# bluemoon-o2/walker-gym

Hardware: AMD Instinct MI355X
Metric: env-steps/sec (whole node) at 65 536 walkers; 1/2/4/8 MI355X scaling (higher is better)
Workload: dtype f32

## Files before the change

include/walker_hip.h:

```cpp
#ifndef WALKER_HIP_H
#define WALKER_HIP_H
#include <stdint.h>

#ifdef __cplusplus
extern "C" {
#endif

typedef struct ihipStream_t *hipStream_t;
typedef struct ihipEvent_t *hipEvent_t;

#define WG_ABI_VERSION 16
#define WG_EINVAL (-1)
#define WG_ERANGE (-2)
#define WG_EHIP (-3)

typedef struct wg_params {
    double g, dampk, ground, groundk, grounddamp, friction, dt;
    double pk, vk, ak, mk;
    int32_t in3d, max_steps;
    int32_t midform;
    int32_t conmid;
    int32_t spring_mode;
    int32_t action_mode;
    int32_t integrator;
// ... 136 lines not shown
    int32_t n_sets, obs_dim, hidden, act_dim;
    uint64_t seed;
    uint32_t generation;
    float sigma;
    const float *theta;
    float *w1, *b1, *w2, *b2;
} wg_es;

int wg_es_perturb(const wg_es *es, int32_t first_pair, int32_t n_pairs, hipStream_t stream);
int wg_es_update(const wg_es *es, int32_t first_pair, int32_t n_pairs, const float *util, double scale, float lr,
                 double *workspace, float *grad, float *theta_out, hipStream_t stream);

typedef struct wg_range {
    const wg_batch *batch;
    const wg_outputs *outputs;
    int64_t action_offset;
    const int32_t *plan;
    int32_t plan_blocks;
    hipStream_t stream;
} wg_range;

int wg_step_ranges(const wg_range *ranges, int32_t n, const wg_params *p, const float *action, int32_t action_cols,
                   int32_t action_stride, hipEvent_t *events);

int wg_run_ranges(const wg_range *ranges, int32_t n, const wg_params *p, const float *action, int32_t action_cols,
                  int32_t action_stride, int64_t action_step, int32_t n_steps, hipEvent_t *events);

int wg_observe(const wg_batch *b, const wg_params *p, const wg_outputs *o, const int32_t *plan,
               int32_t plan_blocks, hipStream_t stream);

typedef wg_params wg_obs_cfg;
int wg_step_simple(const wg_batch *b, const float *action, const wg_params *p, int32_t n_steps, hipStream_t stream);
int wg_observe_simple(const wg_batch *b, const wg_obs_cfg *cfg, float *obs, float *reward, uint8_t *done,
                      float *centroid, float *energy, hipStream_t stream);

int wg_reset(const wg_batch *b, const wg_params *p, const float *noise, const uint8_t *mask,
             hipStream_t stream);

int wg_reset_noise(const wg_batch *b, const float *noise, hipStream_t stream);

int wg_plan_ragged(const int32_t *mass_off, const int32_t *edge_off, const int32_t *muscle_off,
                   int32_t N, int32_t *plan, int32_t max_blocks);

int wg_plan_waves(const int32_t *mass_off, const int32_t *edge_off, const int32_t *muscle_off,
                  int32_t N, int32_t *plan, int32_t max_tiles);
int wg_wave_edge_passes(int32_t M, int32_t K);

int wg_plan_errors(int32_t clear);

int wg_launch_geometry(const wg_batch *b, wg_launch_info *info);

long long wg_fix_launches(void);

int wg_debug_stamps(unsigned long long *host, int n);

int wg_launch_floor(int32_t mode, int32_t blocks, int32_t threads, const float *in, float *out, int32_t n_launches,
                    hipStream_t stream);

int wg_time_step(const wg_batch *batch, const wg_params *params, const float *action, int32_t action_cols,
                 int32_t action_stride, int64_t action_step, const wg_outputs *out, int32_t n_steps,
                 const int32_t *plan, int32_t plan_blocks, hipStream_t stream, float *ms_per_launch);

#ifdef __cplusplus
}
#endif
#endif
```

walker_gym_amd/_lib.py:

```python
from __future__ import annotations

import ctypes as C
import os
import threading

HERE = os.path.dirname(os.path.abspath(__file__))
LIB_NAME = "libwalker_hip.so"
LIB_PATH = os.path.join(HERE, LIB_NAME)
ABI_VERSION = 16

WG_EINVAL, WG_ERANGE, WG_EHIP = -1, -2, -3

_vp = C.c_void_p


class WgParams(C.Structure):
    _fields_ = [(n, C.c_double) for n in ("g", "dampk", "ground", "groundk", "grounddamp", "friction", "dt",
                                           "pk", "vk", "ak", "mk")] + \
               [(n, C.c_int32) for n in ("in3d", "max_steps", "midform", "conmid", "spring_mode", "action_mode",
                                         "integrator", "pair_mode")] + \
               [(n, C.c_double) for n in ("pair_g", "pair_k", "pair_e", "bounce_k")] + \
               [("g3_gravity", C.c_double * 3)] + \
               [(n, C.c_double) for n in ("g3_damping", "g3_air", "g3_ground_level", "g3_restitution",
                                          "g3_friction")] + [("g3_ground", C.c_int32), ("friction_mode", C.c_int32),
# ... 15 lines not shown
                ("reset_noise", _vp), ("reset_noise_rows", C.c_int32), ("reset_noise_stride", C.c_int64),
                ("episodes", _vp)]


class WgOutputs(C.Structure):
    _fields_ = [("obs", _vp), ("obs_stride", C.c_int32), ("reward", _vp), ("done", _vp),
                ("centroid", _vp), ("energy", _vp), ("obs_step", C.c_int64), ("out_step", C.c_int64),
                ("obs_pad_clean", C.c_int32), ("steps", _vp), ("nonfinite", _vp), ("momentum", _vp),
                ("reset", _vp), ("final_obs", _vp)]


class WgRange(C.Structure):
    _fields_ = [("batch", C.POINTER(WgBatch)), ("outputs", C.POINTER(WgOutputs)), ("action_offset", C.c_int64),
                ("plan", _vp), ("plan_blocks", C.c_int32), ("stream", _vp)]


class WgLaunchInfo(C.Structure):
    _fields_ = [("threads", C.c_int32), ("walkers_per_block", C.c_int32), ("blocks", C.c_int32),
                ("lds_bytes", C.c_int32)]


class WgPolicy(C.Structure):
    _fields_ = [("n_sets", C.c_int32), ("obs_dim", C.c_int32), ("hidden", C.c_int32), ("act_dim", C.c_int32),
                ("w1", _vp), ("b1", _vp), ("w2", _vp), ("b2", _vp), ("act_limit", C.c_float),
                ("action_out", _vp), ("action_out_step", C.c_int64), ("return_out", _vp), ("length_out", _vp)]


class WgEpisodeStats(C.Structure):
    _fields_ = [("return_sum", _vp), ("length_sum", _vp), ("episodes_done", _vp), ("tail_return", _vp),
                ("tail_length", _vp), ("ep_return", _vp), ("ep_length", _vp), ("ep_slots", C.c_int32)]


class WgEs(C.Structure):
    _fields_ = [("n_sets", C.c_int32), ("obs_dim", C.c_int32), ("hidden", C.c_int32), ("act_dim", C.c_int32),
                ("seed", C.c_uint64), ("generation", C.c_uint32), ("sigma", C.c_float), ("theta", _vp),
                ("w1", _vp), ("b1", _vp), ("w2", _vp), ("b2", _vp)]


class WgActionNoise(C.Structure):
    _fields_ = [("seed", C.c_uint64), ("step_base", C.c_uint32), ("walker_base", C.c_uint32), ("sigma", _vp),
                ("raw_out", _vp), ("raw_out_step", C.c_int64), ("eps_out", _vp), ("eps_out_step", C.c_int64)]


class WgPolicyRows(C.Structure):
    _fields_ = [("x", _vp), ("x_step", C.c_int64), ("mask", _vp), ("mask_step", C.c_int64), ("n_steps", C.c_int32),
                ("N", C.c_int32)]


POLICY_GRAD_MAX_K = 16384

EXPORTS = ("wg_abi_version", "wg_last_error", "wg_step", "wg_step_ranges", "wg_run_ranges", "wg_rollout", "wg_observe",
           "wg_step_simple", "wg_observe_simple", "wg_reset", "wg_reset_noise", "wg_plan_ragged", "wg_plan_waves",
           "wg_wave_edge_passes", "wg_plan_errors", "wg_launch_geometry", "wg_launch_floor", "wg_time_step",
           "wg_rollout_policy", "wg_rollout_episodes", "wg_fix_launches", "wg_es_perturb", "wg_es_update",
           "wg_rollout_stochastic", "wg_gae", "wg_policy_forward", "wg_policy_backward_workspace", "wg_policy_backward")

_lib = None
_lock = threading.Lock()


class WalkerHipError(RuntimeError):
    pass


def load(path: str | None = None):
    global _lib
    with _lock:
        if _lib is not None:
            return _lib
        p = path or os.environ.get("WALKER_HIP_LIB", LIB_PATH)
        if not os.path.exists(p):
            raise WalkerHipError(
                f"{p} not found: build it with `python -m walker_gym_amd.build` (hipcc --offload-arch=gfx950); "
                "walker_gym_amd has no CPU fallback")
        L = C.CDLL(p)
        L.wg_abi_version.restype = C.c_int
        L.wg_last_error.restype = C.c_char_p
        L.wg_step.argtypes = [C.POINTER(WgBatch), C.POINTER(WgParams), _vp, C.c_int32, C.c_int32, C.c_int64,
                              C.POINTER(WgOutputs), C.c_int32, _vp, C.c_int32, _vp]
        L.wg_rollout.argtypes = L.wg_step.argtypes
        L.wg_rollout_policy.argtypes = [C.POINTER(WgBatch), C.POINTER(WgParams), C.POINTER(WgPolicy),
                                        C.POINTER(WgOutputs), C.c_int32, _vp]
        L.wg_rollout_episodes.argtypes = [C.POINTER(WgBatch), C.POINTER(WgParams), C.POINTER(WgPolicy),
                                          C.POINTER(WgOutputs), C.POINTER(WgEpisodeStats), C.c_int32, _vp]
        L.wg_rollout_stochastic.argtypes = [C.POINTER(WgBatch), C.POINTER(WgParams), C.POINTER(WgPolicy),
                                            C.POINTER(WgActionNoise), C.POINTER(WgOutputs), C.POINTER(WgEpisodeStats),
                                            C.c_int32, _vp]
        L.wg_gae.argtypes = [_vp, _vp, _vp, _vp, _vp, C.c_int32, C.c_int32, C.c_int64, C.c_float, C.c_float, _vp, _vp,
                             _vp]
        L.wg_policy_forward.argtypes = [C.POINTER(WgPolicy), C.POINTER(WgPolicyRows), _vp, C.c_int64, _vp]
        L.wg_policy_backward_workspace.argtypes = [C.POINTER(WgPolicy), C.POINTER(WgPolicyRows), C.c_int32]
        L.wg_policy_backward.argtypes = [C.POINTER(WgPolicy), C.POINTER(WgPolicyRows), _vp, C.c_int64, C.c_int32, _vp,
                                         _vp, _vp, _vp, _vp, _vp]
        L.wg_es_perturb.argtypes = [C.POINTER(WgEs), C.c_int32, C.c_int32, _vp]
        L.wg_es_update.argtypes = [C.POINTER(WgEs), C.c_int32, C.c_int32, _vp, C.c_double, C.c_float, _vp, _vp, _vp, _vp]
        L.wg_step_ranges.argtypes = [C.POINTER(WgRange), C.c_int32, C.POINTER(WgParams), _vp, C.c_int32, C.c_int32,
                                     C.POINTER(_vp)]
        L.wg_run_ranges.argtypes = [C.POINTER(WgRange), C.c_int32, C.POINTER(WgParams), _vp, C.c_int32, C.c_int32,
                                    C.c_int64, C.c_int32, C.POINTER(_vp)]
        L.wg_observe.argtypes = [C.POINTER(WgBatch), C.POINTER(WgParams), C.POINTER(WgOutputs), _vp, C.c_int32, _vp]
        L.wg_step_simple.argtypes = [C.POINTER(WgBatch), _vp, C.POINTER(WgParams), C.c_int32, _vp]
        L.wg_observe_simple.argtypes = [C.POINTER(WgBatch), C.POINTER(WgParams), _vp, _vp, _vp, _vp, _vp, _vp]
        L.wg_reset.argtypes = [C.POINTER(WgBatch), C.POINTER(WgParams), _vp, _vp, _vp]
        L.wg_reset_noise.argtypes = [C.POINTER(WgBatch), _vp, _vp]
        L.wg_plan_ragged.argtypes = [_vp, _vp, _vp, C.c_int32, _vp, C.c_int32]
        L.wg_plan_waves.argtypes = [_vp, _vp, _vp, C.c_int32, _vp, C.c_int32]
        L.wg_wave_edge_passes.argtypes = [C.c_int32, C.c_int32]
        L.wg_plan_errors.argtypes = [C.c_int32]
        L.wg_launch_geometry.argtypes = [C.POINTER(WgBatch), C.POINTER(WgLaunchInfo)]
        L.wg_launch_floor.argtypes = [C.c_int32, C.c_int32, C.c_int32, _vp, _vp, C.c_int32, _vp]
        L.wg_time_step.argtypes = L.wg_step.argtypes + [C.POINTER(C.c_float)]
        for f in EXPORTS[2:]:
            getattr(L, f).restype = C.c_int
        L.wg_fix_launches.restype = C.c_longlong
        L.wg_policy_backward_workspace.restype = C.c_int64
        v = L.wg_abi_version()
        if v != ABI_VERSION:
            raise WalkerHipError(f"{p}: ABI version {v}, expected {ABI_VERSION}")
        _lib = L
        return L


def ptr(t):
    return None if t is None else C.c_void_p(t.data_ptr())


def check(rc: int, what: str) -> int:
    if rc < 0:
        msg = load().wg_last_error().decode(errors="replace")
        exc = ValueError if rc in (WG_EINVAL, WG_ERANGE) else WalkerHipError
        raise exc(f"{what}: {msg} (code {rc})")
    return rc
```

walker_gym_amd/csrc/walker_hip.hip:

```cpp

#include <hip/hip_runtime.h>
#include <hip/hip_ext.h>

#include <algorithm>
#include <atomic>
#include <cstdarg>
#include <cstdint>
#include <cstdio>
#include <cstdlib>
#include <cstring>
#include <type_traits>
#include <vector>

#include "walker_hip.h"
#include "powf2.h"
#include "walker_internal.h"
#include "wg_philox.h"

static thread_local char g_err[512] = "";

int wg_fail(int code, const char *fmt, ...) {
    va_list ap;
    va_start(ap, fmt);
    vsnprintf(g_err, sizeof g_err, fmt, ap);
// ... 1896 lines not shown
        const double e = (b.charge && is_mass) ? b.charge[pl] : kp.pair_e;
        pair_central(kp.pair_k, e, p3, mf, lane, M, is_mass, ax, ay, az, true);
    }
}



typedef TermsAoS LeanTerms;
__device__ __forceinline__ LeanTerms lean_terms(char *sl, const LeanGeo &lg) {
    return TermsAoS{reinterpret_cast<double *>(sl), reinterpret_cast<float *>(sl + lg.off_df)};
}

template <bool IN3D, bool FIX = false>
__device__ __forceinline__ void lean_obs_rows(float *obs, int stride, const KParams &kp, int M, int A, int w0, int wl,
                                              int q, int mu_wl, int mu_ua, bool mass_on, bool mus_on, float px, float py,
                                              float pz, float vx, float vy, float vz, float ax, float ay, float az,
                                              float sx, float sy, float sz, float midx, float midy, float midz, float x) {
    constexpr int d = IN3D ? 3 : 2, per = 3 * d;
    const int nmid = (!FIX && kp.conmid) ? 3 : 0;
    typedef float fvd __attribute__((ext_vector_type(d), aligned(4)));
    if (mass_on) {
        const uint32_t row0 = (uint32_t)(w0 + wl) * (uint32_t)stride;
        const bool sums = !FIX && kp.midform == 2;
        const float mm[3] = {sums ? sx : midx, sums ? sy : midy, sums ? sz : midz};
        const float pm[3] = {px, py, pz}, vm[3] = {vx, vy, vz}, am[3] = {ax, ay, az};
        fvd vp, vv, va;
#pragma unroll
        for (int c = 0; c < d; c++) {
            if constexpr (FIX) {
                vp[c] = pm[c] - mm[c]; vv[c] = vm[c]; va[c] = am[c];
            } else {
                vp[c] = kp.midform ? (pm[c] - mm[c]) * kp.pk : pm[c] * kp.pk;
                vv[c] = vm[c] * kp.vk;
                va[c] = am[c] * kp.ak;
            }
        }
        float *dst = WG_ST(obs, row0 + per * q, 1);
        *reinterpret_cast<fvd *>(dst) = vp;
        *reinterpret_cast<fvd *>(dst + d) = vv;
        *reinterpret_cast<fvd *>(dst + 2 * d) = va;
        if (q == 0) {
            if (nmid) {
                float *mrow = WG_ST(obs, row0 + per * M, 1);
                mrow[0] = kp.midform ? mm[0] : 0.f; mrow[1] = kp.midform ? mm[1] : 0.f;
                mrow[2] = kp.midform ? mm[2] : 0.f;
            }
            for (int r = per * M + nmid + A; r < stride; r++) *WG_ST(obs, row0 + r, 1) = 0.f;
        }
    }
    if (mus_on)
        *WG_ST(obs, (uint32_t)(w0 + mu_wl) * (uint32_t)stride + per * M + nmid + mu_ua, 1) = FIX ? x : x * kp.mk;
}

__device__ __forceinline__ KParams lean_fix_params(KParams kp) {
    kp.pk = 1.f; kp.vk = 1.f; kp.ak = 1.f; kp.mk = 1.f;
    kp.midform = 1; kp.conmid = 0; kp.action_mode = 0; kp.integrator = 0; kp.pair_mode = 0;
    return kp;
}
struct LeanPolOut { float ax, ay, az, sx, sy, sz, reward; int done; int reset; };
template <bool IN3D, int NE, bool RES = false, bool E8 = false, bool AR = false, bool POL = false, bool FIX = false>
__device__ __forceinline__ void lean_compute(const wg_batch &b, const KParams &kp_in, const KOut &o,
                                             const LeanGeo &lg, char *sl, const LeanTile &t, int lane,
                                             LeanIn<NE, E8> &L, bool last = true, const KReset &ar = KReset{},
                                             LeanPolOut *po = nullptr, uint32_t *epw = nullptr, int epw_stride = 1) {
    static_assert(!FIX || (E8 && !RES && !AR && !POL && NE <= 4), "FIX: the plain E8 step instance");
    const KParams kp_fix = FIX ? lean_fix_params(kp_in) : KParams{};
    const KParams &kp = FIX ? kp_fix : kp_in;
    const bool store = !RES || last;
    const int M = b.M, K = b.K, A = b.A;
    const int w0 = t.w0, nE = t.nE;
    const int wl = t.wl, q = t.q, mu_wl = t.mu_wl, mu_ua = t.mu_ua;
    const bool is_mass = FIX || t.is_mass, is_mus = t.is_mus, acts = FIX ? t.is_mus : t.acts;
    const uint32_t pl = t.P0 + lane, ul = t.U0 + lane;
    const LeanTerms ts = lean_terms(sl, lg);
    STAMP_WAVE(t.w0 / lg.wpw);
    uint32_t *s_inc = reinterpret_cast<uint32_t *>(sl + lg.off_inc);
    float *s_x = reinterpret_cast<float *>(sl + lg.off_x);
    const float mf = L.mf;
    const bool pin = !FIX && L.pin != 0;
    double sq_tl = 0.0, sq_te = 0.0;
    if (NE == 1 && !RES) {
        sq_tl = PW_LOG2_TAB[lane & 31];
        sq_te = pw_asdouble(PW_EXP2_TAB[lane & 31]);
    }

    if (!RES) {
        WG_INC_TO_LDS(s_inc, L.gi, lane, nE, NE, FIX);
        if (lane == 0) s_inc[nE] = 0u;
    }
    float x = L.x;
    if (acts) {
        x = muscle_act(kp.action_mode, x, L.a, L.stp, L.lo, L.hi);
        if (store) *WG_ST(b.muscle_x, ul, 1) = x;
    }
    if (is_mus) s_x[lane] = x;
    double ym = recip_m(mf);
    if (!RES) asm volatile("" : "+v"(ym));
    wave_sync();
    STAMP(2);

    bool dead = false;
    if ((!RES || NE == 1) && kp.pair_mode == 0) {
        const bool nanp = is_mass && (__builtin_isnan(L.p3[0]) || __builtin_isnan(L.p3[1]) || __builtin_isnan(L.p3[2]));
        if (__builtin_expect(__ballot(nanp) != 0ull, 0)) {
            const unsigned long long db = __ballot(nanp && !pin && L.io1 > L.io0);
            const unsigned long long gm = (M == 64) ? ~0ull : (((1ull << M) - 1ull) << (lane & ~(M - 1)));
            dead = is_mass && (db & gm) == gm;
            if (dead) {
                L.p3[0] = (float)q; L.p3[1] = 0.f; L.p3[2] = 0.f;
                L.v3[0] = 0.f; L.v3[1] = 0.f; L.v3[2] = 0.f;
            }
        }
    }

    bool gtiny = false;
    const bool pos_ok = __all(fexp3(L.p3[0], L.p3[1], L.p3[2]) >= -55);
    struct Gath { float v[12]; };
    auto gather = [&](int it, Gath &g) {
// ... 51 lines not shown
            const int le = lane + 64 * it;
            if (le < nE) ts.put(le, 0.0, 0.0, 0.0, 0.f, 0.f, 0.f);
            continue;
        }
        Gath g;
        gather(it, g);
        spring(it, g);
    }
    wave_sync();
    const bool wave_tiny = __any(gtiny);
    STAMP(3);

    EnvTerms et{};
    if (!RES) et = env_terms(kp, mf, (float)ym, L.v3[0], L.v3[1], L.v3[2]);
    float px = 0.f, py = 0.f, pz = 0.f, vx = 0.f, vy = 0.f, vz = 0.f, ax = 0.f, ay = 0.f, az = 0.f;
    float nv = 0.f, ke = 0.f, pe = 0.f;
    bool hit = false;
    if (is_mass) {
        const int r1 = (WG_ABLATE & 2) ? min(L.io1, L.io0 + 1) : L.io1;
        const int lb = wl * K;
        if (!RES)
            mass_accumulate_v2(ts, reinterpret_cast<const uint16_t *>(s_inc) + 2 * lb, lb, L.io0, r1, mf, ym, ax, ay, az,
                               wave_tiny);
        else
            mass_accumulate<LeanTerms, !RES>(ts, reinterpret_cast<const uint16_t *>(s_inc) + 2 * lb, lb, L.io0, r1, mf,
                                             ax, ay, az, 0, wave_tiny);
    }
    if (!RES && kp.pair_mode) pair_forces(b, kp, L.p3, mf, pl, lane, M, is_mass, ax, ay, az);
    if (is_mass) {
        mass_tail(kp, mf, (float)ym, L.p3, L.v3, px, py, pz, vx, vy, vz, ax, ay, az, hit, pin,
                  !RES ? &et : nullptr);
        if (dead) nan_state(px, py, pz, vx, vy, vz, ax, ay, az, hit);
        if (!FIX && b.radius && store) b.radius[pl] = hit ? 3.0 : 1.0;
        nv = np_norm3(vx, vy, vz);
        if (!(NE == 1 && !RES)) ke = dead ? nv : mf * np_sq<NE == 1>(nv);
        pe = (float)((double)mf * kp.g) * (py - kp.ground);
    }
    if (NE == 1 && !RES) {
        const float sq = np_sq_wave(dead ? 0.f : nv, sq_tl, sq_te);
        if (is_mass) ke = dead ? nv : mf * sq;
    }
    STAMP(4);

    const int gbase = lane & ~(M - 1);
    const WalkerSums ws = (WG_ABLATE & 4) ? WalkerSums{px, py, pz, py, nv, ke, pe}
                                          : walker_sums(px, py, pz, nv, ke, pe, gbase, M, lane);
    const float sx = ws.sx, sy = ws.sy, sz = ws.sz, ysum = ws.ysum, vsum = ws.vsum, ksum = ws.ksum, psum = ws.psum;
    const unsigned long long gmask = (M == 64) ? ~0ull : (((1ull << M) - 1ull) << gbase);
    const unsigned long long hb = __ballot(is_mass && (py - kp.ground < 0.f));
    const unsigned long long sb = __ballot(is_mass && nv < 0.1f);
    const float midx = sx * lg.invM, midy = sy * lg.invM, midz = sz * lg.invM;
    int ep_done = 0;
    if (is_mass) {
        if (store) WG_STORE_STATE(b, pl, px, py, pz, vx, vy, vz, ax, ay, az, RES || kp.keep_aux, hit)
        if (q == 0) {
            const uint32_t wg = (uint32_t)(w0 + wl);
            const int steps = L.wsteps + 1;
            if (store) *WG_ST(b.steps, wg, 1) = steps;
            if (RES) L.wsteps = steps;
            if (o.steps) *WG_ST(o.steps, wg, 1) = steps;
            const float cy = ysum * lg.invM;
            if constexpr (POL) {
                const float vpen = (-(vsum * lg.invM)) * 0.1f;
                po->reward = (cy + vpen) + neg_half_count((int)__popcll(hb & gmask));
                if (o.reward) *WG_ST(o.reward, wg, 1) = po->reward;
            } else if (FIX || o.reward) {
                const float vpen = (-(vsum * lg.invM)) * 0.1f;
                *WG_ST(o.reward, wg, 1) = (cy + vpen) + neg_half_count((int)__popcll(hb & gmask));
            }
            if (FIX || o.done || (AR && (ar.mode & 1)) || POL) {
                int done;
                WG_EPISODE_DONE(done, steps, cy, (sb & gmask) == gmask, kp);
                if (FIX || o.done) at_u32w(o.done, wg) = (uint8_t)done;
                ep_done = done;
            }
            if (FIX || o.centroid) {
                float *c = WG_ST(o.centroid, wg, 3);
                c[0] = midx; c[1] = midy; c[2] = midz;
            }
            if (FIX || o.energy) *WG_ST(o.energy, wg, 1) = 0.5f * ksum + psum;
        }
    }

    STAMP(5);
    if ((FIX || o.obs) && !(WG_ABLATE & 16))
        lean_obs_rows<IN3D, FIX>(o.obs, o.obs_stride, kp, M, A, w0, wl, q, mu_wl, mu_ua, is_mass, is_mus, px, py, pz,
                                 vx, vy, vz, ax, ay, az, sx, sy, sz, midx, midy, midz, x);
    float rsx = sx, rsy = sy, rsz = sz;
    if constexpr (AR) {
        const bool nonf = is_mass && !(__builtin_isfinite(px) && __builtin_isfinite(py) && __builtin_isfinite(pz) &&
                                       __builtin_isfinite(vx) && __builtin_isfinite(vy) && __builtin_isfinite(vz) &&
                                       __builtin_isfinite(ax) && __builtin_isfinite(ay) && __builtin_isfinite(az));
        const unsigned long long eb = __ballot(is_mass && q == 0 && ep_done != 0), nb = __ballot(nonf);
        const unsigned long long hot = ((ar.mode & 1) ? eb : 0ull) | ((ar.mode & 2) ? nb : 0ull);
        const bool selw = is_mass && (hot & gmask) != 0ull;
        if (ar.reset && is_mass && q == 0) at_u32w(ar.reset, (uint32_t)(w0 + wl)) = (uint8_t)selw;
        if constexpr (POL) po->reset = selw;
        if (__builtin_expect(hot != 0ull, 0)) {
            const unsigned long long mmask = (M == 64) ? ~0ull : (((1ull << M) - 1ull) << ((mu_wl << lg.lgM) & 63));
            const bool selm = is_mus && (hot & mmask) != 0ull;
            if (ar.final_obs)
                lean_obs_rows<IN3D>(ar.final_obs, o.obs_stride, kp, M, A, w0, wl, q, mu_wl, mu_ua, selw, selm, px, py, pz,
                                    vx, vy, vz, ax, ay, az, sx, sy, sz, midx, midy, midz, x);
            int ep = 0;
            if (selw && q == 0) ep = RES ? (int)epw[wl * epw_stride] : at_u32(b.episodes, 4u * (uint32_t)(w0 + wl));
            ep = __builtin_amdgcn_ds_bpermute(gbase << 2, ep);
            float fx = px, fy = py, fz = pz, fvx = vx, fvy = vy, fvz = vz, fax = ax, fay = ay, faz = az, fxm = x;
            if (selw) {
                const float *ip = &at_u32(b.init_pos, 12u * pl), *iv = &at_u32(b.init_vel, 12u * pl),
                            *ia = &at_u32(b.init_acc, 12u * pl);
                fx = ip[0]; fy = ip[1]; fz = ip[2];
                fvx = iv[0]; fvy = iv[1]; fvz = iv[2];
                fax = ia[0]; fay = ia[1]; faz = ia[2];
                if (b.reset_noise) {
                    const float *nz = b.reset_noise +
                                      (size_t)((uint32_t)ep % (uint32_t)b.reset_noise_rows) * (size_t)b.reset_noise_stride +
                                      3 * (size_t)pl;
                    fvx = fvx + nz[0]; fvy = fvy + nz[1];
                    if (IN3D) fvz = fvz + nz[2];
                }
                if (store) {
                    float *gpo = WG_ST(b.pos, pl, 3), *gvo = WG_ST(b.vel, pl, 3), *gao = WG_ST(b.acc, pl, 3);
                    gpo[0] = fx; gpo[1] = fy; gpo[2] = fz;
                    gvo[0] = fvx; gvo[1] = fvy; gvo[2] = fvz;
                    gao[0] = fax; gao[1] = fay; gao[2] = faz;
                }
                if (q == 0) {
                    const uint32_t wg = (uint32_t)(w0 + wl);
                    if (store) *WG_ST(b.steps, wg, 1) = 0;
                    *WG_ST(b.episodes, wg, 1) = ep + 1;
                    if constexpr (RES) {
                        epw[wl * epw_stride] = (uint32_t)(ep + 1);
                        L.wsteps = 0;
                    }
                }
            }
            if (selm) {
                fxm = at_u32(b.init_muscle_x, 4u * ul);
                *WG_ST(b.muscle_x, ul, 1) = fxm;
            }
            if (o.obs && !(WG_ABLATE & 16)) {
                const WalkerSums fs = walker_sums(fx, fy, fz, 0.f, 0.f, 0.f, gbase, M, lane);
                lean_obs_rows<IN3D>(o.obs, o.obs_stride, kp, M, A, w0, wl, q, mu_wl, mu_ua, selw, selm, fx, fy, fz, fvx,
                                    fvy, fvz, fax, fay, faz, fs.sx, fs.sy, fs.sz, fs.sx * lg.invM, fs.sy * lg.invM,
                                    fs.sz * lg.invM, fxm);
            }
            if constexpr (RES) {
                px = fx; py = fy; pz = fz; vx = fvx; vy = fvy; vz = fvz; x = fxm;
                if constexpr (POL) {
                    const WalkerSums fs = walker_sums(fx, fy, fz, 0.f, 0.f, 0.f, gbase, M, lane);
                    ax = fax; ay = fay; az = faz;
                    if (selw) { rsx = fs.sx; rsy = fs.sy; rsz = fs.sz; }
                }
            }
        }
    }
    if (RES) {
        L.p3[0] = px; L.p3[1] = py; L.p3[2] = pz;
        L.v3[0] = vx; L.v3[1] = vy; L.v3[2] = vz;
        L.x = x;
    }
    if constexpr (POL) {
        po->ax = ax; po->ay = ay; po->az = az;
        po->sx = rsx; po->sy = rsy; po->sz = rsz;
        po->done = ep_done;
    }
    STAMP(6);
    STAMP_HW(lane);
}

constexpr int lean_waves(int NE) { return NE >= 8 ? 4 : 6; }

template <bool IN3D, int NE, bool E8, bool AR = false, bool FIX = false>
__global__ __launch_bounds__(256) __attribute__((amdgpu_waves_per_eu(lean_waves(NE)))) void walker_step_lean(
    typename std::conditional<AR, wg_batch, KBatch15>::type bk, KParams kp, const float *__restrict__ action,
    int action_cols, int action_stride, KOut o, LeanGeo lg, typename std::conditional<AR, KReset, KNoReset>::type ar) {
    extern __shared__ __attribute__((aligned(16))) char smem[];
    const wg_batch b = batch_of(bk);
    const int lane = threadIdx.x & 63, wv = __builtin_amdgcn_readfirstlane(threadIdx.x >> 6);
    const int blk = (kp.xcd & 2) ? xcd_block(blockIdx.x, gridDim.x) : (int)blockIdx.x;
    const int tile = blk * lg.wpb + wv;
    if (tile * lg.wpw >= b.N) return;
    STAMP_WAVE(tile);
    STAMP(0);
    const LeanTile t = lean_tile_of<FIX>(b, action, action_cols, lg, tile, lane);
    LeanIn<NE, E8> L;
    if (kp.prio) __builtin_amdgcn_s_setprio(2);
    lean_load<NE, E8, FIX>(b, kp, action, action_stride, t, lane, L);
    if (kp.prio) __builtin_amdgcn_s_setprio(0);
    STAMP(1);
    if constexpr (AR) lean_compute<IN3D, NE, false, E8, true>(b, kp, o, lg, smem + wv * lg.slice, t, lane, L, true, ar);
    else lean_compute<IN3D, NE, false, E8, false, false, FIX>(b, kp, o, lg, smem + wv * lg.slice, t, lane, L);
}

template <bool IN3D, bool E8, bool AR = false, bool FIX = false>
__global__ __launch_bounds__(256) __attribute__((amdgpu_waves_per_eu(lean_waves(1)))) void walker_step_lean1(
    float *pos, float *vel, const void *edges, const uint16_t *inc, int N, int M, int K, int wpw, int wpb, int nblkx,
    wg_batch b, KParams kp, const float *__restrict__ action, int action_cols, int action_stride, KOut o, LeanGeo lg,
    typename std::conditional<AR, KReset, KNoReset>::type ar) {
    extern __shared__ __attribute__((aligned(16))) char smem[];
    b.pos = pos; b.vel = vel; b.inc = inc; b.N = N; b.M = M; b.K = K;
    if (E8) b.edges8 = static_cast<const wg_edge8 *>(edges);
    else b.edges = static_cast<const wg_edge *>(edges);
    lg.nblk = nblkx & 0x3fffffff; lg.wpw = wpw; lg.wpb = wpb;
    kp.prio = (int)((unsigned)nblkx >> 31);
    const int lane = threadIdx.x & 63, wv = __builtin_amdgcn_readfirstlane(threadIdx.x >> 6);
    const int bid = blockIdx.x, xb = xcd_block(bid, lg.nblk);
    const int blk = (nblkx & 0x40000000) ? xb : bid;
    const int tile = blk * lg.wpb + wv;
    if (tile * lg.wpw >= b.N) return;
    STAMP_WAVE(tile);
    STAMP(0);
    const LeanTile t = lean_tile_of<FIX>(b, action, action_cols, lg, tile, lane);
    LeanIn<1, E8> L;
    if (kp.prio) __builtin_amdgcn_s_setprio(2);
    lean_load<1, E8, FIX>(b, kp, action, action_stride, t, lane, L);
    if (kp.prio) __builtin_amdgcn_s_setprio(0);
    STAMP(1);
    if constexpr (AR) lean_compute<IN3D, 1, false, E8, true>(b, kp, o, lg, smem + wv * lg.slice, t, lane, L, true, ar);
    else lean_compute<IN3D, 1, false, E8, false, false, FIX>(b, kp, o, lg, smem + wv * lg.slice, t, lane, L);
}

struct KResetRes {
    KReset r;
    int off_ep;
};
__device__ __forceinline__ KReset kreset_at(const KReset &r, const KOut &o, int s) {
    KReset as = r;
    if (as.reset) as.reset += (size_t)s * o.out_step;
    if (as.final_obs) as.final_obs += (size_t)s * o.obs_step;
    return as;
}
#define WG_KOUT_AT(os, o, s)                                          \
    KOut os = o;                                                      \
    if (os.obs) os.obs += (size_t)s * os.obs_step;                    \
    if (os.reward) os.reward += (size_t)s * os.out_step;              \
    if (os.done) os.done += (size_t)s * os.out_step;                  \
    if (os.energy) os.energy += (size_t)s * os.out_step;              \
    if (os.centroid) os.centroid += 3 * (size_t)s * os.out_step;      \
    if (os.steps) os.steps += (size_t)s * os.out_step
#define WG_PIN_STATIC(L, NE, E8)                                                                                      \
    {                                                                                                                 \
        asm volatile("" : "+v"(L.mf), "+v"(L.io0), "+v"(L.io1), "+v"(L.lo), "+v"(L.hi), "+v"(L.stp));                 \
        _Pragma("unroll") for (int it = 0; it < NE; it++) {                                                           \
            if constexpr (E8) asm volatile("" : "+v"(L.er[it].w), "+v"(L.er[it].rest));                               \
// ... 776 lines not shown
}

int wg_plan_waves(const int32_t *mass_off, const int32_t *edge_off, const int32_t *muscle_off, int32_t N,
                  int32_t *plan, int32_t max_tiles) {
    if (!mass_off || !edge_off || !muscle_off || !plan || N < 0 || max_tiles < 1)
        return wg_fail(WG_EINVAL, "bad plan args");
    int Mmax = 1, Kmax = 0;
    for (int w = 0; w < N; w++) {
        Mmax = std::max(Mmax, mass_off[w + 1] - mass_off[w]);
        Kmax = std::max(Kmax, edge_off[w + 1] - edge_off[w]);
    }
    const int ne = wave_passes(Mmax, Kmax);
    if (!ne) return wg_fail(WG_EINVAL, "a walker does not fit one wave (M=%d K=%d)", Mmax, Kmax);
    return pack_plan(mass_off, edge_off, muscle_off, N, plan, max_tiles, PackCaps{64, 64 * ne, 64, RW_MAXW}, true, "tiles");
}

int wg_plan_ragged(const int32_t *mass_off, const int32_t *edge_off, const int32_t *muscle_off,
                   int32_t N, int32_t *plan, int32_t max_blocks) {
    if (!mass_off || !edge_off || !muscle_off || !plan || N < 0 || max_blocks < 1)
        return wg_fail(WG_EINVAL, "bad plan args");
    return pack_plan(mass_off, edge_off, muscle_off, N, plan, max_blocks, PackCaps{RAG_P, RAG_E, RAG_U, RAG_W}, false,
                     "blocks");
}

int wg_launch_floor(int32_t mode, int32_t blocks, int32_t threads, const float *in, float *out, int32_t n_launches,
                    hipStream_t stream) {
    if (blocks < 1 || threads < 1 || threads > 1024 || n_launches < 0 || mode < 0 || mode > 2 ||
        (mode >= 1 && (!in || !out)))
        return wg_fail(WG_EINVAL, "bad floor launch (mode %d, %d x %d)", mode, blocks, threads);
    for (int i = 0; i < n_launches; i++) {
        if (mode == 0)
            hipLaunchKernelGGL(floor_empty_kernel, dim3(blocks), dim3(threads), 0, stream, out);
        else if (mode == 1)
            hipLaunchKernelGGL(floor_load_store_kernel, dim3(blocks), dim3(threads), 0, stream, in, out);
        else
            hipLaunchKernelGGL(floor_busy_kernel, dim3(blocks), dim3(threads), 0, stream, in, out);
    }
    return hipGetLastError() == hipSuccess ? 0 : wg_fail(WG_EHIP, "floor launch failed");
}

int wg_debug_stamps(unsigned long long *host, int n) {
#ifdef WG_STAMPS
    if (hipMemcpyFromSymbol(host, HIP_SYMBOL(g_stamps), (size_t)n * 8 * sizeof(unsigned long long), 0,
                            hipMemcpyDeviceToHost) != hipSuccess)
        return wg_fail(WG_EHIP, "stamp copy failed");
    return 0;
#else
    (void)host; (void)n;
    return wg_fail(WG_EINVAL, "not a stamps build");
#endif
}

long long wg_fix_launches(void) { return g_fix_launches.load(std::memory_order_relaxed); }

int wg_launch_geometry(const wg_batch *b, wg_launch_info *info) {
    int rc = validate(b);
    if (rc) return rc;
    if (!info) return wg_fail(WG_EINVAL, "null info");
    LeanGeo lg{};
    if (lean_geo(b, 0, &lg)) {
        info->threads = 64 * lg.wpb;
        info->walkers_per_block = lg.wpb * lg.wpw;
        info->blocks = lg.nblk;
        info->lds_bytes = lg.wpb * lg.slice;
        return 0;
    }
    RagGeo rg{};
    if (b->ragged == 2 && lean_enabled() && rag_geo(b, 0, &rg)) {
        info->threads = 64 * rg.wpb;
        info->walkers_per_block = -1;
        info->blocks = -1;
        info->lds_bytes = rg.wpb * rg.slice;
        return 0;
    }
    const Geo g = b->ragged ? ragged_geo(b) : uniform_geo(b, 0);
    info->threads = g.threads;
    info->walkers_per_block = g.W;
    info->blocks = b->ragged ? -1 : (b->N + g.W - 1) / g.W;
    info->lds_bytes = g.lds;
    return 0;
}

}
```

walker_gym_amd/csrc/wg_host.h:

```cpp
#pragma once

int env_int(const char *name, int dflt) {
    const char *e = getenv(name);
    return (e && *e) ? atoi(e) : dflt;
}

KParams make_kparams(const wg_params &p) {
    KParams k;
    k.neg_g = (float)(-p.g);
    k.neg_dampk = (float)(-p.dampk);
    k.ground = (float)p.ground;
    k.neg_groundk = (float)(-p.groundk);
    k.neg_grounddamp = (float)(-p.grounddamp);
    k.friction = (float)p.friction;
    k.dt = (float)p.dt;
    k.pk = (float)p.pk; k.vk = (float)p.vk; k.ak = (float)p.ak; k.mk = (float)p.mk;
    k.done_y = (float)(p.ground - 50.0);
    k.g = p.g;
    k.max_steps = p.max_steps; k.midform = p.midform; k.conmid = p.conmid;
    k.spring_mode = p.spring_mode; k.action_mode = p.action_mode;
    k.integrator = p.integrator;
    k.pair_mode = p.pair_mode;
    k.pair_g = p.pair_g;
    k.pair_k = p.pair_k;
// ... 166 lines not shown

int lean1_nblkx(const LeanGeo &g, const KParams &kp) {
    return (int)((unsigned)g.nblk | ((unsigned)(kp.xcd & 2) << 29) | ((unsigned)(kp.prio != 0) << 31));
}

template <class F>
void with_flag(bool v, F &&f) {
    if (v) f(std::true_type{});
    else f(std::false_type{});
}
template <class F>
void with_passes(int ne, F &&f) {
    if (ne <= 1) f(std::integral_constant<int, 1>{});
    else if (ne == 2) f(std::integral_constant<int, 2>{});
    else if (ne == 3) f(std::integral_constant<int, 3>{});
    else if (ne == 4) f(std::integral_constant<int, 4>{});
    else f(std::integral_constant<int, 8>{});
}
template <class F>
void with_instance(bool in3d, int ne, F &&f) {
    with_flag(in3d, [&](auto d3) { with_passes(ne, [&](auto n) { f(d3, n); }); });
}
template <class F>
void with_instance(bool in3d, int ne, bool e8, F &&f) {
    with_instance(in3d, ne, [&](auto d3, auto n) { with_flag(e8, [&](auto c8) { f(d3, n, c8); }); });
}

struct Actions {
    const float *ptr;
    int32_t cols, stride;
    int64_t step;
    Actions at(int s) const { return Actions{ptr ? ptr + s * step : nullptr, cols, stride, step}; }
};

bool lean_fix_ok(const wg_batch *b, const KParams &kp, const Actions &a, const wg_outputs &o, const LeanGeo &g, bool e8,
                 int ne, int ar_mode) {
#ifdef WG_STAMPS
    return false;
#endif
    if (WG_ABLATE != 0 || env_int("WG_FIX", 1) == 0) return false;
    auto one = [](float f) {
        uint32_t u;
        memcpy(&u, &f, sizeof u);
        return u == 0x3f800000u;
    };
    return e8 && ne >= 1 && ne <= 4 && ar_mode == 0 && b->N % g.wpw == 0 && g.wpw * b->M == 64 &&
           b->A >= 1 && a.ptr != nullptr && a.cols >= b->A && a.stride >= b->A && kp.action_mode == 0 &&
           kp.pair_mode == 0 && !b->pinned && !b->radius && kp.integrator != 2 && kp.midform == 1 && kp.conmid == 0 &&
           one(kp.pk) && one(kp.vk) && one(kp.ak) && one(kp.mk) &&
           o.obs && o.reward && o.done && o.centroid && o.energy;
}
std::atomic<long long> g_fix_launches{0};

int launch_lean(const wg_batch *b, const KParams &kp, bool in3d, const Actions &a, const wg_outputs &o, const LeanGeo &g,
                hipStream_t st, int ar_mode = 0) {
    const int ne = lean_passes(g, b);
    const uint32_t lds = (uint32_t)(g.wpb * g.slice + std::max(0, env_int("WG_LDS_PAD", 0)));
    const bool e8 = use_edge8(b, g);
    const bool fix = lean_fix_ok(b, kp, a, o, g, e8, ne, ar_mode);
    const dim3 grid(g.nblk), block(64 * g.wpb);
    with_instance(in3d, ne, e8, [&](auto d3, auto n, auto c8) {
        constexpr bool D3 = decltype(d3)::value, E8 = decltype(c8)::value;
        constexpr int NE = decltype(n)::value;
        if constexpr (NE == 1) {
            const void *recs = E8 ? static_cast<const void *>(b->edges8) : static_cast<const void *>(b->edges);
            auto go = [&](auto kernel, auto reset) {
                WG_KLAUNCH(kernel, grid, block, lds, st, b->pos, b->vel, recs, b->inc, b->N, b->M, b->K, g.wpw, g.wpb,
                           lean1_nblkx(g, kp), *b, kp, a.ptr, a.cols, a.stride, kout(o), g, reset);
            };
            if constexpr (E8) {
                if (fix) return go(walker_step_lean1<D3, true, false, true>, KNoReset{});
            }
            if (ar_mode) go(walker_step_lean1<D3, E8, true>, kreset(o, ar_mode));
            else go(walker_step_lean1<D3, E8>, KNoReset{});
        } else {
            auto go = [&](auto kernel, const auto &batch, auto reset) {
                WG_KLAUNCH(kernel, grid, block, lds, st, batch, kp, a.ptr, a.cols, a.stride, kout(o), g, reset);
            };
            if constexpr (E8 && NE <= 4) {
                if (fix) return go(walker_step_lean<D3, NE, true, false, true>, kbatch15(b), KNoReset{});
            }
            if (ar_mode) go(walker_step_lean<D3, NE, E8, true>, *b, kreset(o, ar_mode));
            else go(walker_step_lean<D3, NE, E8>, kbatch15(b), KNoReset{});
        }
    });
    if (const int rc = wg_launched("launch")) return rc;
    if (fix) g_fix_launches.fetch_add(1, std::memory_order_relaxed);
    return 0;
}

int launch_lean_rollout(const wg_batch *b, const KParams &kp, bool in3d, const Actions &a, const wg_outputs &o,
                        int n_steps, const LeanGeo &g0, hipStream_t st, int ar_mode = 0) {
    LeanGeo g = g0;
    const KResetRes ar{kreset(o, ar_mode), g.slice};
    if (ar_mode) g.slice += align16(g.wpw * 4);
    const dim3 grid(g.nblk), block(64 * g.wpb);
    const int lds = g.wpb * g.slice;
    with_instance(in3d, lean_passes(g, b), use_edge8(b, g), [&](auto d3, auto n, auto c8) {
        constexpr bool D3 = decltype(d3)::value, E8 = decltype(c8)::value;
        constexpr int NE = decltype(n)::value;
        if (ar_mode)
            hipLaunchKernelGGL((walker_rollout_lean<D3, NE, E8, true>), grid, block, lds, st, *b, kp, a.ptr, a.cols,
                               a.stride, a.step, kout(o), n_steps, g, ar);
        else
            hipLaunchKernelGGL((walker_rollout_lean<D3, NE, E8>), grid, block, lds, st, *b, kp, a.ptr, a.cols, a.stride,
                               a.step, kout(o), n_steps, g, KNoReset{});
    });
    return wg_launched("launch");
}

int check_auto_reset(const wg_batch *b, int ar_mode) {
    if (ar_mode & ~3) return wg_fail(WG_EINVAL, "auto_reset %d: bits 1 (done) and 2 (non-finite) only", ar_mode);
    if (!b->init_pos || !b->init_vel || !b->init_acc || !b->init_muscle_x)
        return wg_fail(WG_EINVAL, "auto_reset needs the snapshot (init_pos, init_vel, init_acc, init_muscle_x)");
    if (!b->episodes) return wg_fail(WG_EINVAL, "auto_reset needs the episodes array");
    if (b->reset_noise && b->reset_noise_rows < 1)
        return wg_fail(WG_EINVAL, "auto_reset: reset_noise with reset_noise_rows %d < 1", b->reset_noise_rows);
    if (b->reset_noise && b->reset_noise_stride < 3ll * b->N * b->M)
        return wg_fail(WG_EINVAL, "auto_reset: reset_noise_stride %lld < 3 * P = %lld",
                       (long long)b->reset_noise_stride, 3ll * b->N * b->M);
    return 0;
}
int check_integrator(const wg_params *p) {
    return p->integrator < 0 || p->integrator > 2 ? wg_fail(WG_EINVAL, "integrator must be 0/1 (run1) or 2 (run2)") : 0;
}
int check_muscle_bounds(const wg_batch *b) {
    return b->muscle_bounds ? 0 : wg_fail(WG_EINVAL, "actions need muscle_bounds");
}
int check_discrete(const wg_batch *b, const wg_params *p) {
    return p->action_mode == 1 && !b->muscle_stride ? wg_fail(WG_EINVAL, "discrete actions need muscle_stride") : 0;
}

int obs_row_len(const wg_batch *b, const wg_params *p) {
    return 3 * (p->in3d ? 3 : 2) * b->M + (p->conmid ? 3 : 0) + b->A;
}

int rollout_policy(const wg_batch *b, const wg_params *p, const wg_policy *pol, const wg_outputs *o, int32_t n_steps,
                   hipStream_t stream, bool episodes = false, const wg_episode_stats *st = nullptr,
                   bool stochastic = false, const wg_action_noise *nz = nullptr) {
    const char *fn = stochastic ? "wg_rollout_stochastic" : episodes ? "wg_rollout_episodes" : "wg_rollout_policy";
// ... 270 lines not shown
```

walker_gym_amd/device.py:

```python
from __future__ import annotations

import ctypes as C
import os
from typing import Optional

import numpy as np
import torch

from . import _lib
from .layout import HostLayout, default_radius, refresh_edges8, set_springs


def _to_dev(a: np.ndarray, device) -> torch.Tensor:
    a = np.ascontiguousarray(a)
    if a.dtype == np.uint16:
        t = torch.from_numpy(a.view(np.int16))
    elif a.dtype == np.uint32:
        t = torch.from_numpy(a.view(np.int32))
    else:
        t = torch.from_numpy(a)
    return t.to(device, non_blocking=False).contiguous()


class DeviceBatch:
# ... 166 lines not shown
    def _make_struct(self) -> _lib.WgBatch:
        r = self.ragged
        return _lib.WgBatch(
            N=self.N, M=self.M, K=self.K, A=self.A, ragged=self.ragged_kind if r else 0, row=self._p(self.row),
            mass_off=self._p(self.mass_off) if r else None, edge_off=self._p(self.edge_off) if r else None,
            muscle_off=self._p(self.muscle_off) if r else None,
            pos=self._p(self.pos), vel=self._p(self.vel), acc=self._p(self.acc), mass=self._p(self.mass),
            edges=self._p(self.edges),
            inc=self._p(self.inc) if self.inc is not None else None, inc_off=self._p(self.inc_off),
            muscle_x=self._p(self.muscle_x), muscle_bounds=self._p(self.muscle_bounds),
            muscle_stride=self._p(self.muscle_stride), steps=self._p(self.steps), contact=self._p(self.contact),
            pinned=self._p(self.pinned), charge=self._p(self.charge), radius=self._p(self.radius),
            bounce_set=self._p(self.bounce_set),
            edges8=self._p(self.edges8) if not r else None, kc=(C.c_float * 4)(*self.kc),
            **self._auto_reset_fields())

    def sub_struct(self, w0: int, w1: int) -> _lib.WgBatch:
        if self.ragged:
            raise ValueError("sub_struct: uniform batches only")
        if not 0 <= w0 < w1 <= self.N:
            raise ValueError(f"sub_struct: bad walker range [{w0}, {w1})")
        M, K, A = self.M, self.K, self.A

        def off(t, elems):
            return None if t is None else C.c_void_p(t.data_ptr() + elems * t.element_size())

        return _lib.WgBatch(
            N=w1 - w0, M=M, K=K, A=A, ragged=0, mass_off=None, edge_off=None, muscle_off=None,
            pos=off(self.pos, 3 * M * w0), vel=off(self.vel, 3 * M * w0), acc=off(self.acc, 3 * M * w0),
            mass=off(self.mass, M * w0), edges=off(self.edges, 4 * K * w0),
            inc=off(self.inc, 2 * K * w0) if self.inc is not None else None,
            inc_off=off(self.inc_off, (M + 1) * w0),
            muscle_x=self._p(self.muscle_x) if A == 0 else off(self.muscle_x, A * w0),
            muscle_bounds=self._p(self.muscle_bounds) if A == 0 else off(self.muscle_bounds, 2 * A * w0),
            muscle_stride=self._p(self.muscle_stride) if A == 0 else off(self.muscle_stride, A * w0),
            steps=off(self.steps, w0), contact=off(self.contact, M * w0), pinned=off(self.pinned, M * w0),
            charge=off(self.charge, M * w0), radius=off(self.radius, M * w0), row=None,
            bounce_set=off(self.bounce_set, M * w0),
            edges8=off(self.edges8, 2 * K * w0) if self.edges8 is not None and w0 % (64 // M) == 0 else None,
            kc=(C.c_float * 4)(*self.kc), **self._auto_reset_fields(w0))

    def launch_geometry(self) -> dict:
        info = _lib.WgLaunchInfo()
        _lib.check(_lib.load().wg_launch_geometry(C.byref(self.struct), C.byref(info)), "wg_launch_geometry")
        blocks = info.blocks
        if self.ragged:
            wpb = max(1, info.threads // 64)
            blocks = -(-self.plan_blocks // wpb) if self.ragged_kind == 2 else self.plan_blocks
        geo = dict(threads=info.threads, walkers_per_block=info.walkers_per_block, blocks=blocks,
                   lds_bytes=info.lds_bytes)
        if self.ragged_kind == 2:
            geo["wave_tiles"] = self.plan_blocks
        geo["fix_launches"] = int(_lib.load().wg_fix_launches())
        return geo

    KIND = {"pos": "mass", "vel": "mass", "acc": "mass", "contact": "mass", "radius": "mass", "muscle_x": "muscle",
            "steps": "walker"}

    def state_dict(self) -> dict:
        sd = {k: self.caller(k).clone() for k in self.STATE}
        if self.radius is not None:
            sd["radius"] = self.caller("radius").clone()
        return sd

    def load_state_dict(self, sd: dict) -> None:
        self.version += 1
        for k in self.STATE:
            getattr(self, k).copy_(self.to_stored(self.KIND[k], sd[k].to(self.device)))
        if "radius" in sd:
            self.enable_radius()
            self.radius.copy_(self.to_stored("mass", sd["radius"].to(self.device)))
```

Baseline: 2.150 billion.

## Stage pos/vel/obs tile in LDS and write back with coalesced 128-bit buffer stores

```diff
diff --git a/include/walker_hip.h b/include/walker_hip.h
--- a/include/walker_hip.h
+++ b/include/walker_hip.h
@@ -212,6 +212,8 @@
 
 long long wg_fix_launches(void);
 
+long long wg_wt_launches(void);
+
 int wg_debug_stamps(unsigned long long *host, int n);
 
 int wg_launch_floor(int32_t mode, int32_t blocks, int32_t threads, const float *in, float *out, int32_t n_launches,
diff --git a/walker_gym_amd/_lib.py b/walker_gym_amd/_lib.py
--- a/walker_gym_amd/_lib.py
+++ b/walker_gym_amd/_lib.py
@@ -91,7 +91,7 @@
 EXPORTS = ("wg_abi_version", "wg_last_error", "wg_step", "wg_step_ranges", "wg_run_ranges", "wg_rollout", "wg_observe",
            "wg_step_simple", "wg_observe_simple", "wg_reset", "wg_reset_noise", "wg_plan_ragged", "wg_plan_waves",
            "wg_wave_edge_passes", "wg_plan_errors", "wg_launch_geometry", "wg_launch_floor", "wg_time_step",
-           "wg_rollout_policy", "wg_rollout_episodes", "wg_fix_launches", "wg_es_perturb", "wg_es_update",
+           "wg_rollout_policy", "wg_rollout_episodes", "wg_fix_launches", "wg_wt_launches", "wg_es_perturb", "wg_es_update",
            "wg_rollout_stochastic", "wg_gae", "wg_policy_forward", "wg_policy_backward_workspace", "wg_policy_backward")
 
 _lib = None
@@ -152,6 +152,7 @@
         for f in EXPORTS[2:]:
             getattr(L, f).restype = C.c_int
         L.wg_fix_launches.restype = C.c_longlong
+        L.wg_wt_launches.restype = C.c_longlong
         L.wg_policy_backward_workspace.restype = C.c_int64
         v = L.wg_abi_version()
         if v != ABI_VERSION:
diff --git a/walker_gym_amd/csrc/walker_hip.hip b/walker_gym_amd/csrc/walker_hip.hip
--- a/walker_gym_amd/csrc/walker_hip.hip
+++ b/walker_gym_amd/csrc/walker_hip.hip
@@ -1972,18 +1972,57 @@
         *WG_ST(obs, (uint32_t)(w0 + mu_wl) * (uint32_t)stride + per * M + nmid + mu_ua, 1) = FIX ? x : x * kp.mk;
 }
 
+template <bool IN3D>
+__device__ __forceinline__ void lean_tile_image(const wg_batch &b, const KOut &o, char *sl, int M, int A, int w0, int lane,
+                                                int wl, int q, int mu_wl, int mu_ua, bool is_mus, float px, float py,
+                                                float pz, float vx, float vy, float vz, float ax, float ay, float az,
+                                                float midx, float midy, float midz, float x) {
+    constexpr int d = IN3D ? 3 : 2, per = 3 * d;
+    typedef uint32_t u4 __attribute__((ext_vector_type(4)));
+    const int stride = per * M + A;
+    float *img = reinterpret_cast<float *>(sl);
+    wave_sync();
+    float *ip = img + 3 * lane, *iv = img + 192 + 3 * lane, *ir = img + 384 + wl * stride + per * q;
+    ip[0] = px; ip[1] = py; ip[2] = pz;
+    iv[0] = vx; iv[1] = vy; iv[2] = vz;
+    const float pm[3] = {px - midx, py - midy, pz - midz}, vm[3] = {vx, vy, vz}, am[3] = {ax, ay, az};
+#pragma unroll
+    for (int c = 0; c < d; c++) { ir[c] = pm[c]; ir[d + c] = vm[c]; ir[2 * d + c] = am[c]; }
+    if (is_mus) img[384 + mu_wl * stride + per * M + mu_ua] = x;
+    wave_sync();
+    const u4 *im4 = reinterpret_cast<const u4 *>(sl);
+    const uint32_t tile = (uint32_t)w0 >> (6 - (31 - __builtin_clz(M)));
+    const uint32_t nrow = (64u / (uint32_t)M) * (uint32_t)stride * 4u;
+    const uint32_t lb = 16u * (uint32_t)lane;
+    auto put = [&](float *base, uint32_t bytes, uint32_t off, const u4 &v) {
+        const __amdgpu_buffer_rsrc_t rs = __builtin_amdgcn_make_buffer_rsrc(base, 0, (int)bytes, 0x00020000);
+        __builtin_amdgcn_raw_buffer_store_b128(v, rs, (int)off, 0, 16);
+    };
+    const uint32_t sbytes = (uint32_t)b.N * (uint32_t)M * 12u, obytes = (uint32_t)b.N * (uint32_t)stride * 4u;
+    if (lane < 48) {
+        const u4 vp = im4[lane], vv = im4[48 + lane];
+        put(b.pos, sbytes, tile * 768u + lb, vp);
+        put(b.vel, sbytes, tile * 768u + lb, vv);
+    }
+#pragma unroll
+    for (int k = 0; k < 3; k++)
+        if (lb + 1024u * k < nrow) put(o.obs, obytes, tile * nrow + lb + 1024u * k, im4[96 + lane + 64 * k]);
+}
+
 __device__ __forceinline__ KParams lean_fix_params(KParams kp) {
     kp.pk = 1.f; kp.vk = 1.f; kp.ak = 1.f; kp.mk = 1.f;
     kp.midform = 1; kp.conmid = 0; kp.action_mode = 0; kp.integrator = 0; kp.pair_mode = 0;
     return kp;
 }
 struct LeanPolOut { float ax, ay, az, sx, sy, sz, reward; int done; int reset; };
-template <bool IN3D, int NE, bool RES = false, bool E8 = false, bool AR = false, bool POL = false, bool FIX = false>
+template <bool IN3D, int NE, bool RES = false, bool E8 = false, bool AR = false, bool POL = false, bool FIX = false,
+          bool WT = false>
 __device__ __forceinline__ void lean_compute(const wg_batch &b, const KParams &kp_in, const KOut &o,
                                              const LeanGeo &lg, char *sl, const LeanTile &t, int lane,
                                              LeanIn<NE, E8> &L, bool last = true, const KReset &ar = KReset{},
                                              LeanPolOut *po = nullptr, uint32_t *epw = nullptr, int epw_stride = 1) {
     static_assert(!FIX || (E8 && !RES && !AR && !POL && NE <= 4), "FIX: the plain E8 step instance");
+    static_assert(!WT || FIX, "WT: the FIX instances' tile epilogue");
     const KParams kp_fix = FIX ? lean_fix_params(kp_in) : KParams{};
     const KParams &kp = FIX ? kp_fix : kp_in;
     const bool store = !RES || last;
@@ -2141,7 +2180,13 @@
     const float midx = sx * lg.invM, midy = sy * lg.invM, midz = sz * lg.invM;
     int ep_done = 0;
     if (is_mass) {
-        if (store) WG_STORE_STATE(b, pl, px, py, pz, vx, vy, vz, ax, ay, az, RES || kp.keep_aux, hit)
+        if constexpr (WT) {
+            if (kp.keep_aux) {
+                float *gao = WG_ST(b.acc, pl, 3);
+                gao[0] = ax; gao[1] = ay; gao[2] = az;
+                if (b.contact) at_u32w(b.contact, pl) = (uint8_t)hit;
+            }
+        } else if (store) WG_STORE_STATE(b, pl, px, py, pz, vx, vy, vz, ax, ay, az, RES || kp.keep_aux, hit)
         if (q == 0) {
             const uint32_t wg = (uint32_t)(w0 + wl);
             const int steps = L.wsteps + 1;
@@ -2172,7 +2217,10 @@
     }
 
     STAMP(5);
-    if ((FIX || o.obs) && !(WG_ABLATE & 16))
+    if constexpr (WT)
+        lean_tile_image<IN3D>(b, o, sl, M, A, w0, lane, wl, q, mu_wl, mu_ua, is_mus, px, py, pz, vx, vy, vz, ax, ay, az,
+                                  midx, midy, midz, x);
+    else if ((FIX || o.obs) && !(WG_ABLATE & 16))
         lean_obs_rows<IN3D, FIX>(o.obs, o.obs_stride, kp, M, A, w0, wl, q, mu_wl, mu_ua, is_mass, is_mus, px, py, pz,
                                  vx, vy, vz, ax, ay, az, sx, sy, sz, midx, midy, midz, x);
     float rsx = sx, rsy = sy, rsz = sz;
@@ -2260,7 +2308,7 @@
 
 constexpr int lean_waves(int NE) { return NE >= 8 ? 4 : 6; }
 
-template <bool IN3D, int NE, bool E8, bool AR = false, bool FIX = false>
+template <bool IN3D, int NE, bool E8, bool AR = false, bool FIX = false, bool WT = false>
 __global__ __launch_bounds__(256) __attribute__((amdgpu_waves_per_eu(lean_waves(NE)))) void walker_step_lean(
     typename std::conditional<AR, wg_batch, KBatch15>::type bk, KParams kp, const float *__restrict__ action,
     int action_cols, int action_stride, KOut o, LeanGeo lg, typename std::conditional<AR, KReset, KNoReset>::type ar) {
@@ -2279,7 +2327,7 @@
     if (kp.prio) __builtin_amdgcn_s_setprio(0);
     STAMP(1);
     if constexpr (AR) lean_compute<IN3D, NE, false, E8, true>(b, kp, o, lg, smem + wv * lg.slice, t, lane, L, true, ar);
-    else lean_compute<IN3D, NE, false, E8, false, false, FIX>(b, kp, o, lg, smem + wv * lg.slice, t, lane, L);
+    else lean_compute<IN3D, NE, false, E8, false, false, FIX, WT>(b, kp, o, lg, smem + wv * lg.slice, t, lane, L);
 }
 
 template <bool IN3D, bool E8, bool AR = false, bool FIX = false>
@@ -3162,6 +3210,7 @@
 }
 
 long long wg_fix_launches(void) { return g_fix_launches.load(std::memory_order_relaxed); }
+long long wg_wt_launches(void) { return g_wt_launches.load(std::memory_order_relaxed); }
 
 int wg_launch_geometry(const wg_batch *b, wg_launch_info *info) {
     int rc = validate(b);
diff --git a/walker_gym_amd/csrc/wg_host.h b/walker_gym_amd/csrc/wg_host.h
--- a/walker_gym_amd/csrc/wg_host.h
+++ b/walker_gym_amd/csrc/wg_host.h
@@ -242,12 +242,24 @@
 }
 std::atomic<long long> g_fix_launches{0};
 
+bool lean_wt_ok(const wg_batch *b, bool in3d, const wg_outputs &o, const LeanGeo &g, bool fix) {
+    if (!fix || env_int("WG_WT", 1) == 0 || lean_passes(g, b) < 2) return false;
+    const int row = 3 * (in3d ? 3 : 2) * b->M + b->A;
+    const int64_t rows_b = (int64_t)g.wpw * row * 4;
+    auto al16 = [](const void *p) { return (reinterpret_cast<uintptr_t>(p) & 15u) == 0; };
+    static_assert(64 * 12 % 16 == 0, "a tile's pos / vel block");
+    return o.obs_stride == row && al16(b->pos) && al16(b->vel) && al16(o.obs) && rows_b % 16 == 0 &&
+           2 * 768 + rows_b <= g.off_inc;
+}
+std::atomic<long long> g_wt_launches{0};
+
 int launch_lean(const wg_batch *b, const KParams &kp, bool in3d, const Actions &a, const wg_outputs &o, const LeanGeo &g,
                 hipStream_t st, int ar_mode = 0) {
     const int ne = lean_passes(g, b);
     const uint32_t lds = (uint32_t)(g.wpb * g.slice + std::max(0, env_int("WG_LDS_PAD", 0)));
     const bool e8 = use_edge8(b, g);
     const bool fix = lean_fix_ok(b, kp, a, o, g, e8, ne, ar_mode);
+    const bool wt = lean_wt_ok(b, in3d, o, g, fix);
     const dim3 grid(g.nblk), block(64 * g.wpb);
     with_instance(in3d, ne, e8, [&](auto d3, auto n, auto c8) {
         constexpr bool D3 = decltype(d3)::value, E8 = decltype(c8)::value;
@@ -268,6 +280,7 @@
                 WG_KLAUNCH(kernel, grid, block, lds, st, batch, kp, a.ptr, a.cols, a.stride, kout(o), g, reset);
             };
             if constexpr (E8 && NE <= 4) {
+                if (wt) return go(walker_step_lean<D3, NE, true, false, true, true>, kbatch15(b), KNoReset{});
                 if (fix) return go(walker_step_lean<D3, NE, true, false, true>, kbatch15(b), KNoReset{});
             }
             if (ar_mode) go(walker_step_lean<D3, NE, E8, true>, *b, kreset(o, ar_mode));
@@ -276,6 +289,7 @@
     });
     if (const int rc = wg_launched("launch")) return rc;
     if (fix) g_fix_launches.fetch_add(1, std::memory_order_relaxed);
+    if (wt) g_wt_launches.fetch_add(1, std::memory_order_relaxed);
     return 0;
 }
 
diff --git a/walker_gym_amd/device.py b/walker_gym_amd/device.py
--- a/walker_gym_amd/device.py
+++ b/walker_gym_amd/device.py
@@ -242,6 +242,7 @@
         if self.ragged_kind == 2:
             geo["wave_tiles"] = self.plan_blocks
         geo["fix_launches"] = int(_lib.load().wg_fix_launches())
+        geo["wt_launches"] = int(_lib.load().wg_wt_launches())
         return geo
 
     KIND = {"pos": "mass", "vel": "mass", "acc": "mass", "contact": "mass", "radius": "mass", "muscle_x": "muscle",
```

Measured after the change: 2.211 billion, median of 6. 1.03x the previous value.
